# SuperScientificSoftwareLaboratory/DASP

Measured on AMD Instinct MI355X. Metric: SpMV GFLOP/s (f64), higher is better.
Workload: dtype f64; 1 GPU; HV15R synthetic stand-in (seeded; SuiteSparse dims/row statistics), A=1, x=1; rows=2017169, cols=2017169, nnz=275454726, partition=single GPU, generator_rev=26e32ff958e7, y_candidates=1

## Files before the change

### dasp_amd/csrc/spmv_device.hpp

```cpp
#pragma once
#include <hip/hip_runtime.h>

#include <cstdint>

#include "plan.hpp"
#include "device.hpp"

namespace dasp {

typedef double f64x4 __attribute__((ext_vector_type(4)));
typedef double f64x2 __attribute__((ext_vector_type(2)));
typedef float f32x4 __attribute__((ext_vector_type(4)));
typedef _Float16 f16x4 __attribute__((ext_vector_type(4)));
typedef int i32x4 __attribute__((ext_vector_type(4)));
typedef int i32x2 __attribute__((ext_vector_type(2)));
typedef unsigned short u16x4 __attribute__((ext_vector_type(4)));
typedef unsigned short u16x8 __attribute__((ext_vector_type(8)));
typedef const __attribute__((address_space(1))) unsigned char *gbyte_p;
typedef _Float16 f16x8 __attribute__((ext_vector_type(8)));


template <bool NT, class U>
__device__ __forceinline__ U ldg(const U *p)
{
    if constexpr (NT) return __builtin_nontemporal_load(p);
    else return *p;
}

template <int CTRL>
__device__ __forceinline__ double dpp_mov_f64(double v)
{
    int lo = __double2loint(v), hi = __double2hiint(v);
    lo = __builtin_amdgcn_update_dpp(lo, lo, CTRL, 0xf, 0xf, false);
    hi = __builtin_amdgcn_update_dpp(hi, hi, CTRL, 0xf, 0xf, false);
    return __hiloint2double(hi, lo);
}
template <int CTRL>
__device__ __forceinline__ float dpp_mov_f32(float v)
{
    return __int_as_float(__builtin_amdgcn_update_dpp(__float_as_int(v), __float_as_int(v), CTRL, 0xf, 0xf, false));
}
__device__ __forceinline__ double readlane_f64(double v, int l)
{
    int lo = __builtin_amdgcn_readlane(__double2loint(v), l);
    int hi = __builtin_amdgcn_readlane(__double2hiint(v), l);
    return __hiloint2double(hi, lo);
}
__device__ __forceinline__ double wave_sum(double v)
{
    v += dpp_mov_f64<0x128>(v);
    v += dpp_mov_f64<0x124>(v);
    v += dpp_mov_f64<0x122>(v);
    v += dpp_mov_f64<0x121>(v);
    return (readlane_f64(v, 0) + readlane_f64(v, 16)) + (readlane_f64(v, 32) + readlane_f64(v, 48));
}
__device__ __forceinline__ float wave_sum(float v)
{
    v += dpp_mov_f32<0x128>(v);
    v += dpp_mov_f32<0x124>(v);
    v += dpp_mov_f32<0x122>(v);
    v += dpp_mov_f32<0x121>(v);
    float a = __int_as_float(__builtin_amdgcn_readlane(__float_as_int(v), 0));
    float b = __int_as_float(__builtin_amdgcn_readlane(__float_as_int(v), 16));
    float c = __int_as_float(__builtin_amdgcn_readlane(__float_as_int(v), 32));
    float d = __int_as_float(__builtin_amdgcn_readlane(__float_as_int(v), 48));
    return (a + b) + (c + d);
}

template <bool K, class U>
__device__ __forceinline__ U tab(const U *p, int i)
{
    if constexpr (K) return reinterpret_cast<const __attribute__((address_space(4))) U *>(reinterpret_cast<uintptr_t>(p))[i];
    else return p[i];
}

#ifdef DASP_STAMPS
struct CallArgs { const DevArgs *plan; const void *x; void *y; int acc, ywt, stamp_launch; };
#else
struct CallArgs { const DevArgs *plan; const void *x; void *y; int acc, ywt; };
#endif
template <class U> __device__ __forceinline__ U *ldp(U *const *field)
{
    typedef __attribute__((address_space(1))) U *gptr;
    return (U *)*reinterpret_cast<const __attribute__((address_space(4))) gptr *>(reinterpret_cast<uintptr_t>(field));
}
__device__ __forceinline__ DevArgs load_args(const CallArgs &c)
{
    static_assert(sizeof(DevArgs) % 4 == 0, "DevArgs is a whole number of words");
    int w[sizeof(DevArgs) / 4];
#pragma unroll
    for (int i = 0; i < (int)(sizeof(DevArgs) / 4); ++i) w[i] = tab<true>(reinterpret_cast<const int *>(c.plan), i);
    DevArgs a;
    __builtin_memcpy(&a, w, sizeof a);
#define DASP_G(f) a.f = ldp(&c.plan->f)
    DASP_G(long_val); DASP_G(long_cid); DASP_G(long_cid16); DASP_G(long_base); DASP_G(piece_c16); DASP_G(piece_ptr); DASP_G(piece_dst); DASP_G(partial); DASP_G(multi_ptr); DASP_G(multi_dst);
    DASP_G(med_ptr); DASP_G(med_val); DASP_G(med_cid); DASP_G(med_cid16); DASP_G(med_base); DASP_G(med_cid8); DASP_G(med_c8ptr); DASP_G(med_shplane); DASP_G(med_shtab);
    DASP_G(irr_ptr); DASP_G(med_nt); DASP_G(irr_val); DASP_G(irr_cid); DASP_G(med_dst); DASP_G(win_cmin); DASP_G(win_len);
    DASP_G(short_val); DASP_G(short_cid); DASP_G(groups); DASP_G(order);
    DASP_G(rt_val); DASP_G(rt_cid); DASP_G(rt_ptr); DASP_G(rt_start); DASP_G(rt_mask);
#undef DASP_G
    a.x = c.x; a.y = c.y; a.acc = c.acc; a.ywt = c.ywt;
    return a;
}

template <int I, int N> struct LastLE {
    static __device__ __forceinline__ void run(const int (&arr)[N], int w, int &idx, int &val)
    {
        if constexpr (I < N) { const bool in = w >= arr[I]; idx = in ? I : idx; val = in ? arr[I] : val; LastLE<I + 1, N>::run(arr, w, idx, val); }
    }
};
template <int I, int N> struct PickPair {
    static __device__ __forceinline__ void run(const int (&arr)[N], int k, int &lo, int &hi)
    {
        if constexpr (I + 1 < N) { lo = k == I ? arr[I] : lo; hi = k == I ? arr[I + 1] : hi; PickPair<I + 1, N>::run(arr, k, lo, hi); }
    }
};

__device__ __forceinline__ int slot_of(const SlotMap &m, int t)
{
    const int p = t < m.split ? 0 : 1;
    const int u = p ? t - m.split : t;
    const int g = m.grp[p];
    return g ? m.base[p] + (u / g) * 2 * g + m.off[p] + u % g : m.base[p] + u;
}

template <class T> struct Tr;
template <> struct Tr<double> {
    using acc_t = f64x4; using part_t = double;
    static constexpr int CHUNK = 64, SHORT_ROWS = 128, BATCH = kMedBatch64, SHOT = kMedShot64, LONG_SHOT = kMedShot64;
};
template <> struct Tr<_Float16> {
    using acc_t = f32x4; using part_t = float;
    static constexpr int CHUNK = 256, SHORT_ROWS = 256, BATCH = kMedBatch16, SHOT = kMedShot16, LONG_SHOT = 2;
};
static_assert(Tr<double>::BATCH == kMedBatch64 && Tr<double>::SHOT == kMedShot64 && Tr<_Float16>::BATCH == kMedBatch16 &&
              Tr<_Float16>::SHOT == kMedShot16 && kMedBatch64 % 2 == 0 && kMedBatch16 % 2 == 0, "the packers' pairing rule (plan.hpp) follows the kernel's batches");

template <class T> struct Frag;
template <> struct Frag<double> { double a; int c; double b; };
template <> struct Frag<_Float16> { f16x4 a; i32x4 c; f16x4 b; };

template <bool NT>
__device__ __forceinline__ void frag_load_at(Frag<double> &f, const double *val, const int *cid, size_t at)
{
    f.a = ldg<NT>(val + at);
    f.c = ldg<NT>(cid + at);
}
template <bool NT>
__device__ __forceinline__ void frag_load_at(Frag<_Float16> &f, const _Float16 *val, const int *cid, size_t at)
{
    f.a = ldg<NT>(reinterpret_cast<const f16x4 *>(val + at));
    f.c = ldg<NT>(reinterpret_cast<const i32x4 *>(cid + at));
}
template <bool NT, class T>
__device__ __forceinline__ void frag_load(Frag<T> &f, const T *val, const int *cid, size_t e, int lane)
{
    frag_load_at<NT>(f, val, cid, e + (size_t)(Tr<T>::CHUNK / kWave) * lane);
}
template <class T>
struct XGlobal {
    const T *x;
    __device__ __forceinline__ T at(int c) const { return x[c < 0 ? 0 : c]; }
};
template <class T> using lds_cptr = const __attribute__((address_space(3))) T *;
template <class T> using glb_cptr = const __attribute__((address_space(1))) T *;
template <class T>
struct XLds {
    lds_cptr<T> xw; int cmin;
    __device__ __forceinline__ T at(int c) const { return xw[c < 0 ? 0 : c - cmin]; }
};
template <class T>
struct XHyb {
    lds_cptr<T> xw; glb_cptr<T> xg; int cmin; unsigned len;
    __device__ __forceinline__ T at(int c) const
    {
        const unsigned o = (unsigned)(c - cmin);
        T v;
        if (c < 0) v = (T)0;
        else if (o < len) v = xw[o];
        else v = xg[c];
        return v;
    }
};
template <class XV>
__device__ __forceinline__ void frag_gather(Frag<double> &f, const XV &xv)
{
    const double v = xv.at(f.c);
    f.b = f.c < 0 ? 0.0 : v;
}
template <class XV>
__device__ __forceinline__ void frag_gather(Frag<_Float16> &f, const XV &xv)
{
#pragma unroll
    for (int j = 0; j < 4; ++j) {
        const _Float16 v = xv.at(f.c[j]);
        f.b[j] = f.c[j] < 0 ? (_Float16)0 : v;
    }
}
__device__ __forceinline__ void frag_mfma(f64x4 &acc, const Frag<double> &f)
{
    acc = __builtin_amdgcn_mfma_f64_16x16x4f64(f.a, f.b, acc, 0, 0, 0);
}
__device__ __forceinline__ void frag_mfma(f32x4 &acc, const Frag<_Float16> &f)
{
    acc = __builtin_amdgcn_mfma_f32_16x16x16f16(f.a, f.b, acc, 0, 0, 0);
}


template <class T, bool NT>
struct ChunkSrc {
    static constexpr bool kPairs = false, kQuadIds = false;
    const T *val; const int *cid; size_t e0; int lane;
    template <bool PAIRED_OK = true> __device__ __forceinline__ void load(Frag<T> &f, int i) const { frag_load<NT>(f, val, cid, e0 + (size_t)i * Tr<T>::CHUNK, lane); }
    template <bool QUAD = false, class XV> __device__ __forceinline__ void gather(Frag<T> &f, int, const XV &x) const { frag_gather(f, x); }
};

template <class T, bool NT, bool N16 = false>
struct PieceSrc {
    static constexpr bool kPairs = false, kQuadIds = false;
    static constexpr int VPL = Tr<T>::CHUNK / kWave;
    const T *val; const int *cid; size_t e0; int lane, nfull, tail;
    const unsigned short *cid16 = nullptr; const int *base = nullptr;
    template <bool PAIRED_OK = true> __device__ __forceinline__ void load(Frag<T> &f, int i) const
    {
        if constexpr (N16) {
            const size_t at = i < nfull || VPL * lane < tail ? e0 + (size_t)i * Tr<T>::CHUNK + (size_t)(VPL * lane) : e0;
            if constexpr (VPL == 1) { f.a = ldg<NT>(val + at); f.c = (int)ldg<NT>(cid16 + at); }
            else {
                f.a = ldg<NT>(reinterpret_cast<const f16x4 *>(val + at));
                const i32x2 o = ldg<NT>(reinterpret_cast<const i32x2 *>(cid16 + at));
                f.c[0] = o[0]; f.c[1] = o[1];
            }
        } else {
            if (i < nfull) frag_load<NT>(f, val, cid, e0 + (size_t)i * Tr<T>::CHUNK, lane);
            else frag_load_at<NT>(f, val, cid, VPL * lane < tail ? e0 + (size_t)i * Tr<T>::CHUNK + (size_t)(VPL * lane) : e0);
        }
    }
    template <bool QUAD = false, class XV> __device__ __forceinline__ void gather(Frag<T> &f, int i, const XV &x) const
    {
        if constexpr (N16) {
            const int b = tab<true>(base, i);
            if constexpr (VPL == 1) { const unsigned o = (unsigned)f.c; f.c = o == kLongPad16 ? -1 : b + (int)o; }
            else {
                const unsigned lo = (unsigned)f.c[0], hi = (unsigned)f.c[1];
                const unsigned o[4] = {lo & 0xFFFFu, lo >> 16, hi & 0xFFFFu, hi >> 16};
#pragma unroll
                for (int q = 0; q < 4; ++q) f.c[q] = o[q] == kLongPad16 ? -1 : b + (int)o[q];
            }
        }
        if (i >= nfull) {
            const bool ok = VPL * lane < tail;
            if constexpr (VPL == 1) { f.c = ok ? f.c : -1; f.a = ok ? f.a : 0.0; }
            else {
#pragma unroll
                for (int j = 0; j < 4; ++j) { f.c[j] = ok ? f.c[j] : -1; f.a[j] = ok ? f.a[j] : (_Float16)0; }
            }
        }
        frag_gather(f, x);
    }
};

template <class T, bool NT, bool C16, bool PAIRS, bool C8, bool KT = false, bool REL = false, bool SH = false>
struct BlockSrc {
    static constexpr bool kPairs = PAIRS;
    static constexpr int VPL = Tr<T>::CHUNK / kWave;
    ChunkSrc<T, NT> reg; int nc;
    int npair;
    const unsigned short *cid16; const int *base; int c0;
    int relb;
    const unsigned char *c8; const unsigned short *w16; int n8;
    gbyte_p shn, shw; unsigned sh4l, shlane4;
    const T *ival; const int *icid; int t0, t1, kq;
    template <bool PAIRED_OK> __device__ __forceinline__ size_t at_of(int i) const
    {
        constexpr int CH = Tr<T>::CHUNK;
        if constexpr (!PAIRED_OK || !PAIRS) return reg.e0 + (size_t)i * CH + (size_t)VPL * reg.lane;
        const bool paired = i < npair;
        const size_t s = reg.e0 + (paired ? (size_t)(i & ~1) * CH + (size_t)(VPL * (i & 1)) : (size_t)i * CH);
        return s + (size_t)(paired ? 2 * VPL : VPL) * reg.lane;
    }
    __device__ __forceinline__ bool pairs_ok(int i0, int n) const { return i0 + n <= npair; }
    __device__ __forceinline__ void load2(Frag<T> &f0, Frag<T> &f1, int i) const
    {
        constexpr int CH = Tr<T>::CHUNK;
        const size_t at = reg.e0 + (size_t)i * CH + (size_t)(2 * VPL) * reg.lane;
        if constexpr (sizeof(T) == 8) {
            const f64x2 v = ldg<NT>(reinterpret_cast<const f64x2 *>(reg.val + at));
            f0.a = v[0]; f1.a = v[1];
            if constexpr (C16) {
                if constexpr (kQuadIds) {
                    if (i < n8) {
                        const unsigned r = ldg<NT>(reinterpret_cast<const unsigned short *>(c8 + (size_t)i * CH) + reg.lane);
                        const unsigned b0 = r & 0xFFu, b1 = r >> 8;
                        f0.c = (int)(b0 == 0xFFu ? 0xFFFFu : b0); f1.c = (int)(b1 == 0xFFu ? 0xFFFFu : b1);
                        return;
                    }
                }
                const unsigned r = ldg<NT>(reinterpret_cast<const unsigned *>((kQuadIds ? w16 : cid16) + at));
                f0.c = (int)(r & 0xFFFFu); f1.c = (int)(r >> 16);
            } else {
                const i32x2 c = ldg<NT>(reinterpret_cast<const i32x2 *>(reg.cid + at));
                f0.c = c[0]; f1.c = c[1];
            }
        } else {
            const f16x8 v = ldg<NT>(reinterpret_cast<const f16x8 *>(reg.val + at));
            f0.a = __builtin_shufflevector(v, v, 0, 1, 2, 3); f1.a = __builtin_shufflevector(v, v, 4, 5, 6, 7);
            if constexpr (C16) {
                const i32x4 o = ldg<NT>(reinterpret_cast<const i32x4 *>(cid16 + at));
                f0.c[0] = o[0]; f0.c[1] = o[1]; f1.c[0] = o[2]; f1.c[1] = o[3];
            } else {
                f0.c = ldg<NT>(reinterpret_cast<const i32x4 *>(reg.cid + at));
                f1.c = ldg<NT>(reinterpret_cast<const i32x4 *>(reg.cid + at + 4));
            }
        }
    }
    static constexpr bool kQuadIds = C8 && PAIRS && C16 && sizeof(T) == 8 && Tr<T>::BATCH == 4;
    __device__ __forceinline__ void load4(Frag<T> *f, int i) const
    {
        constexpr int CH = Tr<T>::CHUNK;
        const size_t at = reg.e0 + (size_t)i * CH + (size_t)2 * reg.lane;
        const f64x2 v0 = ldg<NT>(reinterpret_cast<const f64x2 *>(reg.val + at));
        const f64x2 v1 = ldg<NT>(reinterpret_cast<const f64x2 *>(reg.val + at + 2 * CH));
        f[0].a = v0[0]; f[1].a = v0[1]; f[2].a = v1[0]; f[3].a = v1[1];
        const bool narrow = i + 4 <= n8;
        gbyte_p pa, pb; unsigned lo4;
        if constexpr (SH) {
            pa = narrow ? shn + (size_t)((unsigned)i * sh4l) : shw + (size_t)((unsigned)i * (2u * sh4l));
            pb = narrow ? pa : pa + 4u * sh4l;
            lo4 = shlane4;
        } else {
            pa = narrow ? (gbyte_p)(c8 + (size_t)i * CH) : (gbyte_p)(w16 + reg.e0 + (size_t)i * CH);
            pb = narrow ? pa : pa + 4 * CH;
            lo4 = 4u * (unsigned)reg.lane;
        }
        const unsigned ra = ldg<NT>((const __attribute__((address_space(1))) unsigned *)(pa + lo4));
        const unsigned rb = ldg<NT>((const __attribute__((address_space(1))) unsigned *)(pb + lo4));
        f[0].c = (int)ra; f[1].c = (int)ra; f[2].c = (int)rb; f[3].c = (int)rb;
    }
    template <bool PAIRED_OK = true> __device__ __forceinline__ void load(Frag<T> &f, int i) const
    {
        if (i < nc) {
            const size_t at = at_of<PAIRED_OK>(i);
            if constexpr (!C16) frag_load_at<NT>(f, reg.val, reg.cid, at);
            else {
                if constexpr (sizeof(T) == 8) {
                    f.a = ldg<NT>(reg.val + at);
                    f.c = (int)ldg<NT>((kQuadIds ? w16 : cid16) + at);
                } else {
                    f.a = ldg<NT>(reinterpret_cast<const f16x4 *>(reg.val + at));
                    const i32x2 o = ldg<NT>(reinterpret_cast<const i32x2 *>(cid16 + at));
                    f.c[0] = o[0]; f.c[1] = o[1];
                }
            }
            return;
        }
        const int j = i - nc;
        if constexpr (sizeof(T) == 8) {
            const int e = t0 + 4 * j + kq;
            const int ee = e < t1 ? e : 0;
            f.a = ldg<NT>(ival + ee);
            f.c = ldg<NT>(icid + ee);
        } else {
#pragma unroll
            for (int q = 0; q < 4; ++q) {
                const int e = t0 + 16 * j + 4 * kq + q;
                const int ee = e < t1 ? e : 0;
                f.a[q] = ival[ee];
                f.c[q] = icid[ee];
            }
        }
    }
    template <bool QUAD = false, class XV> __device__ __forceinline__ void gather(Frag<T> &f, int i, const XV &x) const
    {
        if (i >= nc) {
            const int j = i - nc;
            if constexpr (sizeof(T) == 8) {
                const bool ok = t0 + 4 * j + kq < t1;
                f.a = ok ? f.a : 0.0;
                f.c = ok ? f.c : -1;
            } else {
#pragma unroll
                for (int q = 0; q < 4; ++q) {
                    const bool ok = t0 + 16 * j + 4 * kq + q < t1;
                    f.a[q] = ok ? f.a[q] : (_Float16)0;
                    f.c[q] = ok ? f.c[q] : -1;
                }
            }
        } else if constexpr (C16) {
            const int b = REL ? relb : tab<KT>(base, c0 + i);
            if constexpr (sizeof(T) == 8) {
                unsigned o = (unsigned)f.c, pad = 0xFFFFu;
                if constexpr (QUAD && kQuadIds) {
                    const bool narrow = i < n8, paired = i < npair;
                    pad = narrow ? 0xFFu : 0xFFFFu;
                    o = (o >> (narrow ? 8u * (i & 3) : (paired ? 16u * (i & 1) : 0u))) & pad;
                }
                f.c = o == pad ? -1 : b + (int)o;
            }
            else {
                const unsigned lo = (unsigned)f.c[0], hi = (unsigned)f.c[1];
                const unsigned o[4] = {lo & 0xFFFFu, lo >> 16, hi & 0xFFFFu, hi >> 16};
#pragma unroll
                for (int q = 0; q < 4; ++q) f.c[q] = o[q] == 0xFFFFu ? -1 : b + (int)o[q];
            }
        }
        frag_gather(f, x);
    }
};

template <int N, class SRC, class T>
__device__ __forceinline__ void load_steps(const SRC &src, Frag<T> *f, int i0)
{
    if constexpr (SRC::kPairs && N == Tr<T>::BATCH) {
        if (src.pairs_ok(i0, N)) {
            if constexpr (SRC::kQuadIds) src.load4(f, i0);
            else {
#pragma unroll
                for (int u = 0; u < N; u += 2) src.load2(f[u], f[u + 1], i0 + u);
            }
            return;
        }
    }
#pragma unroll
    for (int u = 0; u < N; ++u) src.load(f[u], i0 + u);
}

template <class T, int N, class SRC, class ACC, class XV>
__device__ __forceinline__ void shot(ACC &acc, const SRC &src, int i0, const XV &x)
{
    Frag<T> f[N];
    if constexpr (SRC::kPairs && sizeof(T) == 2) {
#pragma unroll
        for (int u = 0; u + 1 < N; u += 2) {
            if (src.pairs_ok(i0 + u, 2)) src.load2(f[u], f[u + 1], i0 + u);
            else { src.load(f[u], i0 + u); src.load(f[u + 1], i0 + u + 1); }
        }
        if constexpr (N % 2 == 1) src.load(f[N - 1], i0 + N - 1);
    } else if constexpr (SRC::kPairs && N >= 2) {
        if (src.pairs_ok(i0, N & ~1)) {
#pragma unroll
            for (int u = 0; u + 1 < N; u += 2) src.load2(f[u], f[u + 1], i0 + u);
            if constexpr (N % 2 == 1) src.template load<false>(f[N - 1], i0 + N - 1);
        } else {
#pragma unroll
            for (int u = 0; u < N; ++u) src.template load<false>(f[u], i0 + u);
        }
    } else {
#pragma unroll
        for (int u = 0; u < N; ++u) src.template load<false>(f[u], i0 + u);
    }
#pragma unroll
    for (int u = 0; u < N; ++u) src.gather(f[u], i0 + u, x);
#pragma unroll
    for (int u = 0; u < N; ++u) frag_mfma(acc, f[u]);
}
template <class T, int N, class SRC, class ACC, class XV>
struct ShotDispatch {
    static __device__ __forceinline__ void run(ACC &acc, const SRC &src, int i0, int n, const XV &x)
    {
        if (n == N) shot<T, N>(acc, src, i0, x);
        else ShotDispatch<T, N - 1, SRC, ACC, XV>::run(acc, src, i0, n, x);
    }
};
template <class T, class SRC, class ACC, class XV>
struct ShotDispatch<T, 0, SRC, ACC, XV> {
    static __device__ __forceinline__ void run(ACC &, const SRC &, int, int, const XV &) {}
};

template <class T, int U, int R, class SRC, class ACC, class XV>
struct FinishDispatch {
    static __device__ __forceinline__ void run(ACC &acc, const SRC &src, Frag<T> (&cur)[U], int ibase, int i, int rem, const XV &x)
    {
        if (rem == R) {
            Frag<T> r[R > 0 ? R : 1];
#pragma unroll
            for (int u = 0; u < U; ++u) src.template gather<true>(cur[u], ibase + u, x);
            load_steps<R>(src, r, i);
#pragma unroll
            for (int u = 0; u < U; ++u) frag_mfma(acc, cur[u]);
#pragma unroll
            for (int u = 0; u < R; ++u) src.template gather<true>(r[u], i + u, x);
#pragma unroll
            for (int u = 0; u < R; ++u) frag_mfma(acc, r[u]);
        } else if constexpr (R > 0) FinishDispatch<T, U, R - 1, SRC, ACC, XV>::run(acc, src, cur, ibase, i, rem, x);
    }
};

template <class T, int U, int S, class SRC, class ACC, class XV>
__device__ __forceinline__ void run_stream(ACC &acc, const SRC &src, int N, const XV &x)
{
    if (N <= S) { ShotDispatch<T, S, SRC, ACC, XV>::run(acc, src, 0, N, x); return; }
    const int nfull = N / U, rem = N % U;
    Frag<T> cur[U];
    load_steps<U>(src, cur, 0);
    int i = U;
    for (int it = 1; it < nfull; ++it, i += U) {
        Frag<T> nxt[U];
#pragma unroll
        for (int u = 0; u < U; ++u) src.template gather<true>(cur[u], i - U + u, x);
        load_steps<U>(src, nxt, i);
#pragma unroll
        for (int u = 0; u < U; ++u) frag_mfma(acc, cur[u]);
#pragma unroll
        for (int u = 0; u < U; ++u) cur[u] = nxt[u];
    }
    FinishDispatch<T, U, U - 1, SRC, ACC, XV>::run(acc, src, cur, i - U, i, rem, x);
}

template <class T, int YS = 0, class P>
__device__ __forceinline__ void put_y(const DevArgs &a, int yi, P v)
{
    T *y = static_cast<T *>(a.y) + yi;
    if constexpr (YS == 1) *(volatile T *)y = (T)v;
    else if constexpr (YS == 2) {
        const T old = *(volatile T *)y;
        *(volatile T *)y = (T)((P)old + v);
    }
    else if (a.acc) *y = (T)((P)*y + v);
    else if (a.ywt) *(volatile T *)y = (T)v;
    else *y = (T)v;
}

__device__ __forceinline__ bool diag_of(const f64x4 &acc, int lane, double &d)
{
    const int r = (lane & 15) >> 2;
    d = r == 0 ? acc[0] : r == 1 ? acc[1] : r == 2 ? acc[2] : acc[3];
    return (lane & 3) == (lane >> 4);
}
__device__ __forceinline__ bool diag_of(const f32x4 &acc, int lane, float &d)
{
    const int r = lane & 3;
    d = r == 0 ? acc[0] : r == 1 ? acc[1] : r == 2 ? acc[2] : acc[3];
    return ((lane & 15) >> 2) == (lane >> 4);
}

template <class T, bool NT, bool C16, int YM, bool C8 = false, int YS = 0, bool REL = false, int WU = 0, int WS = 0, bool SH = false, class XV>
__device__ __forceinline__ void medium_block(const DevArgs &a, int b, int lane, const XV &x)
{
    using acc_t = typename Tr<T>::acc_t;
    constexpr int CH = Tr<T>::CHUNK;
    const T *val = static_cast<const T *>(a.med_val);
    constexpr bool KT = true;
    const int c0 = tab<KT>(a.med_ptr, b), c1 = tab<KT>(a.med_ptr, b + 1);
    acc_t acc = {0, 0, 0, 0};
    const int row = lane & 15, kq = lane >> 4;
    const int r = b * kMedRows + row;
    int t0 = 0, t1 = 0;
    if (r < a.row_block) { t0 = a.irr_ptr[r]; t1 = a.irr_ptr[r + 1]; }
    constexpr int TK = sizeof(T) == 8 ? 4 : 16;
    const int nt = YS == 0 ? tab<true>(a.med_nt, b) : (__builtin_amdgcn_readfirstlane(t1 - t0) + TK - 1) / TK;
    BlockSrc<T, NT, C16, YM != 2, C8, KT, REL, SH> src;
    if constexpr (REL) src.relb = x.cmin; else src.relb = 0;
    src.reg.val = val; src.reg.cid = a.med_cid; src.reg.e0 = (size_t)c0 * CH; src.reg.lane = lane;
    src.nc = c1 - c0; src.npair = med_npair(c1 - c0, nt, (int)sizeof(T), YM == 2 ? 0 : a.pair_mode); src.cid16 = a.med_cid16; src.base = a.med_base; src.c0 = c0;
    src.c8 = a.med_cid8; src.w16 = a.med_cid16; src.n8 = 0;
    if constexpr (C8 && C16 && sizeof(T) == 8 && YM != 2) {
        const int q0 = tab<true>(a.med_c8ptr, b), q1 = tab<true>(a.med_c8ptr, b + 1);
        src.n8 = q1 - q0; src.c8 = a.med_cid8 + (size_t)q0 * CH; src.w16 = a.med_cid16 - (size_t)q1 * CH;
    }
    if constexpr (SH) {
        static_assert(C8 && C16 && sizeof(T) == 8 && YM == 0, "the shared id plane belongs to the one-byte-id f64 build");
        typedef unsigned u32x4 __attribute__((ext_vector_type(4)));
        const u32x4 e = tab<true>(reinterpret_cast<const u32x4 *>(a.med_shtab), b);
        const unsigned L = e[3], rw = row < 8 ? e[0] : e[1];
        src.sh4l = 4u * L; src.shlane4 = 4u * ((unsigned)kq * L + ((rw >> (4u * (unsigned)(row & 7))) & 15u));
        src.shn = (gbyte_p)a.med_shplane + (size_t)e[2] * 16;
        src.shw = src.shn - (size_t)((unsigned)src.n8 * src.sh4l);
    }
    src.ival = static_cast<const T *>(a.irr_val); src.icid = a.irr_cid; src.t0 = t0; src.t1 = t1; src.kq = kq;
    run_stream<T, (WU > 0 && sizeof(T) == 8) ? WU : Tr<T>::BATCH, (YM == 2 && sizeof(T) == 2) ? 2 : ((WS > 0 && sizeof(T) == 8) ? WS : Tr<T>::SHOT)>(acc, src, src.nc + nt, x);

    typename Tr<T>::part_t d;
    if (diag_of(acc, lane, d) && r < a.row_block) {
        const int slot = a.row_long + r;
        const int yi = YM == 2 ? a.med_dst[r] : (a.order ? a.order[slot] : slot);
        put_y<T, YS>(a, yi, d);
    }
}

template <class T, bool NT, int YS = 0, bool TAIL_IN = false, bool L16 = false>
__device__ __forceinline__ void long_piece(const DevArgs &a, int p, int lane)
{
    using acc_t = typename Tr<T>::acc_t;
    using part_t = typename Tr<T>::part_t;
    constexpr int CH = Tr<T>::CHUNK;
    constexpr int VPL = CH / kWave;
    const XGlobal<T> x{static_cast<const T *>(a.x)};
    const T *val = static_cast<const T *>(a.long_val);
    const int p0 = tab<true>(a.piece_ptr, p), p1 = tab<true>(a.piece_ptr, p + 1);
    acc_t acc = {0, 0, 0, 0};
    const int nfull = (p1 - p0) / CH, tail = (p1 - p0) - nfull * CH;
    bool narrow = false;
    if constexpr (L16) narrow = tab<true>(a.piece_c16, 2 * p + 1) != 0;
    if (L16 && narrow) {
        const PieceSrc<T, NT, true> src{val, a.long_cid, (size_t)p0, lane, nfull, tail, a.long_cid16, a.long_base + tab<true>(a.piece_c16, 2 * p)};
        run_stream<T, Tr<T>::BATCH, Tr<T>::LONG_SHOT>(acc, src, nfull + (tail > 0 ? 1 : 0), x);
    } else if (TAIL_IN && tail > 0) {
        const PieceSrc<T, NT> src{val, a.long_cid, (size_t)p0, lane, nfull, tail};
        run_stream<T, Tr<T>::BATCH, Tr<T>::LONG_SHOT>(acc, src, nfull + 1, x);
    } else {
        const int full = p0 + nfull * CH;
        ChunkSrc<T, NT> src{val, a.long_cid, (size_t)p0, lane};
        run_stream<T, Tr<T>::BATCH, Tr<T>::LONG_SHOT>(acc, src, nfull, x);
        if (full < p1) {
            const int i = full + VPL * lane;
            const bool ok = i < p1;
            Frag<T> f;
            frag_load_at<NT>(f, val, a.long_cid, (size_t)(ok ? i : p0));
            frag_gather(f, x);
            if constexpr (VPL == 1) { f.a = ok ? f.a : 0.0; f.b = ok ? f.b : 0.0; }
            else {
#pragma unroll
                for (int j = 0; j < 4; ++j) { f.a[j] = ok ? f.a[j] : (_Float16)0; f.b[j] = ok ? f.b[j] : (_Float16)0; }
            }
            frag_mfma(acc, f);
        }
    }
    part_t d;
    const bool on_diag = diag_of(acc, lane, d);
    const part_t total = wave_sum(on_diag ? d : (part_t)0);
    if (lane == 0) {
        const int dst = tab<true>(a.piece_dst, p);
        if (dst >= 0) put_y<T, YS>(a, dst, total);
        else static_cast<part_t *>(a.partial)[~dst] = total;
    }
}

template <class T, int L, bool NT, int YS = 0>
__device__ __forceinline__ void short_rows(const DevArgs &a, const ShortDev &g, int local_tile, int lane)
{
    constexpr int SR = Tr<T>::SHORT_ROWS;
    constexpr int V = SR / kWave;
    const T *x = static_cast<const T *>(a.x);
    const T *val = static_cast<const T *>(a.short_val);
    using part_t = typename Tr<T>::part_t;
    part_t s[V];
#pragma unroll
    for (int v = 0; v < V; ++v) s[v] = 0;
    const size_t base = (size_t)g.elem_off + (size_t)local_tile * L * SR + (size_t)V * lane;
#pragma unroll
    for (int k = 0; k < L; ++k) {
        if constexpr (V == 2) {
            const f64x2 av = ldg<NT>(reinterpret_cast<const f64x2 *>(val + base + (size_t)k * SR));
            const i32x2 c = ldg<NT>(reinterpret_cast<const i32x2 *>(a.short_cid + base + (size_t)k * SR));
            const double x0 = x[c[0] < 0 ? 0 : c[0]], x1 = x[c[1] < 0 ? 0 : c[1]];
            s[0] += av[0] * (c[0] < 0 ? 0.0 : x0);
            s[1] += av[1] * (c[1] < 0 ? 0.0 : x1);
        } else {
            const f16x4 av = ldg<NT>(reinterpret_cast<const f16x4 *>(val + base + (size_t)k * SR));
            const i32x4 c = ldg<NT>(reinterpret_cast<const i32x4 *>(a.short_cid + base + (size_t)k * SR));
#pragma unroll
            for (int v = 0; v < 4; ++v) {
                const _Float16 xv = x[c[v] < 0 ? 0 : c[v]];
                s[v] += (float)av[v] * (c[v] < 0 ? 0.0f : (float)xv);
            }
        }
    }
    const int t0 = local_tile * SR + V * lane;
#pragma unroll
    for (int v = 0; v < V; ++v) {
        const int t = t0 + v;
        if (t < g.count) {
            const int slot = slot_of(g.map, t);
            const int yi = a.order ? a.order[slot] : slot;
            put_y<T, YS>(a, yi, s[v]);
        }
    }
}

template <class T, int L, bool NT, int YS = 0>
__device__ __forceinline__ void short_rows_seg(const DevArgs &a, const ShortDev &g, int local_tile, int lane)
{
    constexpr int PER16 = 16 / L, RPW = 4 * PER16;
    using part_t = typename Tr<T>::part_t;
    const T *x = static_cast<const T *>(a.x);
    const int sub = lane & 15, rloc = sub / L, k = sub - rloc * L;
    const int t = local_tile * RPW + (lane >> 4) * PER16 + rloc;
    const size_t e = (size_t)g.elem_off + (size_t)local_tile * kWave + (size_t)lane;
    const T av = ldg<NT>(static_cast<const T *>(a.short_val) + e);
    const int c = ldg<NT>(a.short_cid + e);
    const T xv = x[c < 0 ? 0 : c];
    part_t p = c < 0 ? (part_t)0 : (part_t)av * (part_t)xv;
    if constexpr (L >= 2) {
        part_t q;
        if constexpr (sizeof(part_t) == 8) q = dpp_mov_f64<0x101>(p); else q = dpp_mov_f32<0x101>(p);
        if (k + 1 < L) p += q;
    }
    if constexpr (L >= 3) {
        part_t q;
        if constexpr (sizeof(part_t) == 8) q = dpp_mov_f64<0x102>(p); else q = dpp_mov_f32<0x102>(p);
        if (k == 0) p += q;
    }
    if (k == 0 && rloc < PER16 && t < g.count) {
        const int slot = slot_of(g.map, t);
        const int yi = a.order ? a.order[slot] : slot;
        put_y<T, YS>(a, yi, p);
    }
}

template <class T, int L, bool NT, int TPW>
__device__ __forceinline__ void short_rows_seg_multi(const DevArgs &a, const ShortDev &g, int local0, int nv, int lane)
{
    constexpr int PER16 = 16 / L, RPW = 4 * PER16;
    using part_t = typename Tr<T>::part_t;
    const T *x = static_cast<const T *>(a.x);
    const int sub = lane & 15, rloc = sub / L, k = sub - rloc * L;
    T av[TPW]; int c[TPW]; T xv[TPW];
#pragma unroll
    for (int u = 0; u < TPW; ++u) {
        const size_t e = (size_t)g.elem_off + (size_t)(local0 + (u < nv ? u : 0)) * kWave + (size_t)lane;
        av[u] = ldg<NT>(static_cast<const T *>(a.short_val) + e);
        c[u] = ldg<NT>(a.short_cid + e);
    }
#pragma unroll
    for (int u = 0; u < TPW; ++u) xv[u] = x[c[u] < 0 ? 0 : c[u]];
#pragma unroll
    for (int u = 0; u < TPW; ++u) {
        part_t p = c[u] < 0 ? (part_t)0 : (part_t)av[u] * (part_t)xv[u];
        if constexpr (L >= 2) {
            part_t q;
            if constexpr (sizeof(part_t) == 8) q = dpp_mov_f64<0x101>(p); else q = dpp_mov_f32<0x101>(p);
            if (k + 1 < L) p += q;
        }
        if constexpr (L >= 3) {
            part_t q;
            if constexpr (sizeof(part_t) == 8) q = dpp_mov_f64<0x102>(p); else q = dpp_mov_f32<0x102>(p);
            if (k == 0) p += q;
        }
        const int t = (local0 + u) * RPW + (lane >> 4) * PER16 + rloc;
        if (u < nv && k == 0 && rloc < PER16 && t < g.count) {
            const int slot = slot_of(g.map, t);
            const int yi = a.order ? a.order[slot] : slot;
            put_y<T>(a, yi, p);
        }
    }
}

template <class T, bool NT, int YS = 0>
__device__ __forceinline__ void slab_rows(const DevArgs &a, const ShortDev &g, int local_tile, int lane)
{
    constexpr int SR = Tr<T>::SHORT_ROWS;
    constexpr int V = SR / kWave;
    const T *x = static_cast<const T *>(a.x);
    const T *val = static_cast<const T *>(a.short_val);
    using part_t = typename Tr<T>::part_t;
    const int L = g.len;
    part_t s[V];
#pragma unroll
    for (int v = 0; v < V; ++v) s[v] = 0;
    const size_t base = (size_t)g.elem_off + (size_t)local_tile * L * SR + (size_t)V * lane;
#pragma unroll 4
    for (int k = 0; k < L; ++k) {
        if constexpr (V == 2) {
            const f64x2 av = ldg<NT>(reinterpret_cast<const f64x2 *>(val + base + (size_t)k * SR));
            const i32x2 c = ldg<NT>(reinterpret_cast<const i32x2 *>(a.short_cid + base + (size_t)k * SR));
            const double x0 = x[c[0] < 0 ? 0 : c[0]], x1 = x[c[1] < 0 ? 0 : c[1]];
            s[0] += av[0] * (c[0] < 0 ? 0.0 : x0);
            s[1] += av[1] * (c[1] < 0 ? 0.0 : x1);
        } else {
            const f16x4 av = ldg<NT>(reinterpret_cast<const f16x4 *>(val + base + (size_t)k * SR));
            const i32x4 c = ldg<NT>(reinterpret_cast<const i32x4 *>(a.short_cid + base + (size_t)k * SR));
#pragma unroll
            for (int v = 0; v < 4; ++v) {
                const _Float16 xv = x[c[v] < 0 ? 0 : c[v]];
                s[v] += (float)av[v] * (c[v] < 0 ? 0.0f : (float)xv);
            }
        }
    }
    const int t0 = local_tile * SR + V * lane;
#pragma unroll
    for (int v = 0; v < V; ++v) {
        const int t = t0 + v;
        if (t < g.count) {
            const int slot = g.map.base[0] + t;
            const int yi = a.order ? a.order[slot] : slot;
            put_y<T, YS>(a, yi, s[v]);
        }
    }
}

template <class T, bool NT, int YS = 0, bool SEG = true>
__device__ __forceinline__ void short_tile(const DevArgs &a, int tile, int lane)
{
    int gi = 0, t0_unused = 0;
    LastLE<1, kNumShortGroups>::run(a.grp_tile0, tile, gi, t0_unused);
    ShortDev g;
    if constexpr (YS != 0) {
        static_assert(sizeof(ShortDev) % 4 == 0, "ShortDev is a whole number of words");
        int w[sizeof(ShortDev) / 4];
#pragma unroll
        for (int i = 0; i < (int)(sizeof(ShortDev) / 4); ++i) w[i] = tab<true>(reinterpret_cast<const int *>(a.groups + gi), i);
        __builtin_memcpy(&g, w, sizeof g);
    } else g = a.groups[gi];
    const int local = tile - g.tile0;
    if constexpr (SEG) {
        if (g.seg) {
            switch (g.len) {
                case 1: short_rows_seg<T, 1, NT, YS>(a, g, local, lane); break;
                case 2: short_rows_seg<T, 2, NT, YS>(a, g, local, lane); break;
                case 3: short_rows_seg<T, 3, NT, YS>(a, g, local, lane); break;
                default: short_rows_seg<T, 4, NT, YS>(a, g, local, lane); break;
            }
            return;
        }
    }
    switch (g.len) {
        case 0: if constexpr (YS != 2) { if (!a.skip0 && !a.acc) short_rows<T, 0, NT, YS>(a, g, local, lane); } break;
        case 1: short_rows<T, 1, NT, YS>(a, g, local, lane); break;
        case 2: short_rows<T, 2, NT, YS>(a, g, local, lane); break;
        case 3: short_rows<T, 3, NT, YS>(a, g, local, lane); break;
        case 4: short_rows<T, 4, NT, YS>(a, g, local, lane); break;
        default: slab_rows<T, NT, YS>(a, g, local, lane); break;
    }
}

template <class T, bool NT, int TPW>
__device__ __forceinline__ void short_waves(const DevArgs &a, int w, int lane)
{
    int gi = 0, w0 = 0;
    LastLE<1, kNumShortGroups>::run(a.grp_wave0, w, gi, w0);
    const ShortDev g = a.groups[gi];
    const int lw = w - w0;
    if (!g.seg) { short_tile<T, NT, 0, false>(a, g.tile0 + lw, lane); return; }
    const int local0 = lw * TPW, nv = min(TPW, g.tiles - local0);
    switch (g.len) {
        case 1: short_rows_seg_multi<T, 1, NT, TPW>(a, g, local0, nv, lane); break;
        case 2: short_rows_seg_multi<T, 2, NT, TPW>(a, g, local0, nv, lane); break;
        case 3: short_rows_seg_multi<T, 3, NT, TPW>(a, g, local0, nv, lane); break;
        default: short_rows_seg_multi<T, 4, NT, TPW>(a, g, local0, nv, lane); break;
    }
}

template <class T, bool NT>
__device__ __forceinline__ void row_tile(const DevArgs &a, int t, int lane, typename Tr<T>::part_t *prod)
{
    using part_t = typename Tr<T>::part_t;
    const T *x = static_cast<const T *>(a.x), *val = static_cast<const T *>(a.rt_val);
    const int e0 = a.rt_ptr[t], n = a.rt_ptr[t + 1] - e0;
    const int s = a.rt_start[(size_t)t * kRowTile + lane];
#pragma unroll 4
    for (int i = lane; i < n; i += kWave) prod[i] = (part_t)ldg<NT>(val + e0 + i) * (part_t)x[ldg<NT>(a.rt_cid + e0 + i)];
    int e = __shfl_down(s, 1);
    if (lane == kWave - 1) e = n;
    part_t sum = 0;
    for (int j = s; j < e; ++j) sum += prod[j];
    if ((a.rt_mask[t] >> lane) & 1) put_y<T>(a, t * kRowTile + lane, sum);
}

#ifdef DASP_STAMPS
struct StampBuf { unsigned long long *rec; unsigned cap; };
static __device__ StampBuf g_stamps;
struct Stamps {
    unsigned long long wall0, clk[4];
    int kind, launch;
    __device__ __forceinline__ void begin(int launch_no) { wall0 = __builtin_amdgcn_s_memrealtime(); clk[0] = __builtin_readcyclecounter(); clk[1] = clk[2] = clk[3] = clk[0]; kind = 0; launch = launch_no; }
    __device__ __forceinline__ void mark(int i) { asm volatile("s_waitcnt vmcnt(0) lgkmcnt(0)" ::: "memory"); clk[i] = __builtin_readcyclecounter(); }
    __device__ __forceinline__ void finish(int nwaves)
    {
        asm volatile("s_waitcnt vmcnt(0) lgkmcnt(0)" ::: "memory");
        const unsigned long long e = __builtin_readcyclecounter();
        const unsigned long long wall1 = __builtin_amdgcn_s_memrealtime();
        const size_t slot = ((size_t)launch * gridDim.x + blockIdx.x) * (size_t)nwaves + (threadIdx.x >> 6);
        if ((threadIdx.x & 63) == 0 && g_stamps.rec && launch >= 0 && slot < g_stamps.cap) {
            unsigned long long *r = g_stamps.rec + slot * 12;
            unsigned xcc, hw;
            asm volatile("s_getreg_b32 %0, hwreg(HW_REG_XCC_ID)" : "=s"(xcc));
            asm volatile("s_getreg_b32 %0, hwreg(HW_REG_HW_ID)" : "=s"(hw));
            r[0] = blockIdx.x | ((unsigned long long)(threadIdx.x >> 6) << 32) | ((unsigned long long)nwaves << 40) | ((unsigned long long)kind << 48) | (1ull << 63);
            r[1] = xcc | ((unsigned long long)hw << 32); r[2] = gridDim.x; r[3] = wall0; r[4] = wall1;
            r[5] = clk[0]; r[6] = clk[1]; r[7] = clk[2]; r[8] = clk[3]; r[9] = e; r[10] = (unsigned long long)launch; r[11] = 0;
        }
    }
};
#else
struct Stamps {
    int kind;
    __device__ __forceinline__ void begin(int) {}
    __device__ __forceinline__ void mark(int) {}
};
#endif

#ifndef DASP_MIN_WAVES
#define DASP_MIN_WAVES 1
#endif
constexpr int kMinWavesPlain = DASP_MIN_WAVES, kMinWavesWin = 8;
#ifndef DASP_WIN64_U
#define DASP_WIN64_U 3
#define DASP_WIN64_S 6
#endif
template <class T, bool NT, bool C16, bool WIN, bool C8, bool RT = false, bool W64 = false, bool L16 = false, bool SH = false>
__device__ __forceinline__ void spmv_body(const DevArgs &a, char *lds_raw, int wg_index, Stamps &st)
{
    const int lane = threadIdx.x & 63;
    const int wave = __builtin_amdgcn_readfirstlane(threadIdx.x >> 6);
    int wg = wg_index;
    if constexpr (sizeof(T) == 2 && !WIN && !RT) {
        if (a.wg_rot) { const int grid = a.wg_long + a.wg_med + a.wg_short; wg += a.wg_rot; wg = wg >= grid ? wg - grid : wg; }
    }
    const int wpw = WIN ? a.wpw : kWavesPerWG;
    if (wg < a.wg_long) {
        const int p = wg * wpw + wave;
        if (p < a.n_pieces) long_piece<T, NT, 0, !WIN, L16 && !WIN>(a, p, lane);
    } else if (wg < a.wg_long + a.wg_med) {
        st.kind = 1;
        if constexpr (!WIN) {
            const int m = wg - a.wg_long;
            const XGlobal<T> x{static_cast<const T *>(a.x)};
            if (a.xcd_on) {
                const int k = m & 7;
                int lo = a.xcd_blk[0], hi = a.xcd_blk[1];
                PickPair<1, 9>::run(a.xcd_blk, k, lo, hi);
                const int b = lo + (m >> 3) * kWavesPerWG + wave;
                if (b < hi) medium_block<T, NT, C16, 0, C8, 0, false, 0, 0, SH>(a, b, lane, x);
            } else if (sizeof(T) == 8 && !a.med_stride) {
                const int b = m * kWavesPerWG + wave;
                if (b < a.n_blocks) medium_block<T, NT, C16, 0, C8, 0, false, 0, 0, SH>(a, b, lane, x);
            } else {
#pragma unroll 1
            for (int b = m * kWavesPerWG + wave; b < a.n_blocks; b += a.wg_med * kWavesPerWG)
                medium_block<T, NT, C16, 0, C8, 0, false, 0, 0, SH>(a, b, lane, x);
            }
        } else {
            const int mw = wg - a.wg_long, per_xcd = a.wg_med >> 3;
            const int w = a.win_xcd ? (mw & 7) * per_xcd + (mw >> 3) : mw;
            if (w >= a.n_windows) return;
            const int len = a.win_len[w], cmin = a.win_cmin[w];
            const T *xg = static_cast<const T *>(a.x);
            __shared__ int next_unit_word;
            int *next_unit = &next_unit_word;
            typedef __attribute__((address_space(3))) T lds_T;
            lds_T *xw = (lds_T *)lds_raw;
            if (threadIdx.x == 0) *next_unit = wpw;
            st.kind = 3; st.mark(1);
            if (len > 0) {
                constexpr int A = 16 / (int)sizeof(T);
                const i32x4 *src = reinterpret_cast<const i32x4 *>(xg + cmin);
                typedef __attribute__((address_space(3))) i32x4 lds_i32x4;
                lds_i32x4 *dst = (lds_i32x4 *)xw;
                const int nvec = len / A, nth = wpw * kWave;
                for (int i0 = threadIdx.x; i0 < nvec; i0 += 4 * nth) {
                    const int i1 = i0 + nth, i2 = i0 + 2 * nth, i3 = i0 + 3 * nth;
                    const i32x4 v0 = src[i0];
                    const i32x4 v1 = src[i1 < nvec ? i1 : i0], v2 = src[i2 < nvec ? i2 : i0], v3 = src[i3 < nvec ? i3 : i0];
                    dst[i0] = v0;
                    if (i1 < nvec) dst[i1] = v1;
                    if (i2 < nvec) dst[i2] = v2;
                    if (i3 < nvec) dst[i3] = v3;
                }
                for (int i = nvec * A + threadIdx.x; i < len; i += nth) xw[i] = xg[cmin + i];
                st.mark(2);
            }
            __syncthreads();
            st.mark(3);
            const int n_units = a.blocks_per_win + a.win_tiles;
            constexpr int WU = W64 ? DASP_WIN64_U : 0, WS = W64 ? DASP_WIN64_S : 0;
            int q = wave;
#define DASP_NEXT_UNIT()                                                                                          \
            {                                                                                                     \
                int nq = 0;                                                                                       \
                if (lane == 0) nq = atomicAdd(next_unit, 1);                                                      \
                q = __builtin_amdgcn_readfirstlane(nq);                                                           \
            }
#define DASP_WINDOW_BLOCKS(BLOCK_CALL)                                                                            \
            while (q < a.blocks_per_win) {                                                                        \
                const int b = w * a.blocks_per_win + q;                                                           \
                if (b < a.n_blocks) { BLOCK_CALL; }                                                               \
                DASP_NEXT_UNIT()                                                                                  \
            }
            if (len > 0) {
                if (a.win_hybrid) {
                    const XHyb<T> x{xw, (glb_cptr<T>)xg, cmin, (unsigned)len};
                    DASP_WINDOW_BLOCKS((medium_block<T, NT, C16, 2, false, 0, false, WU, WS>(a, b, lane, x)))
                } else if (C16 && a.win_rel16) {
                    const XLds<T> x{xw, cmin};
#ifdef DASP_WIN_KEEPMOD
                    if ((w % DASP_WIN_KEEPMOD) != DASP_WIN_KEEPMOD - 1) { DASP_WINDOW_BLOCKS((medium_block<T, false, C16, 2, false, 0, C16, WU, WS>(a, b, lane, x))) }
                    else
#endif
                    DASP_WINDOW_BLOCKS((medium_block<T, NT, C16, 2, false, 0, C16, WU, WS>(a, b, lane, x)))
                } else {
                    const XLds<T> x{xw, cmin};
                    DASP_WINDOW_BLOCKS((medium_block<T, NT, C16, 2, false, 0, false, WU, WS>(a, b, lane, x)))
                }
            } else {
                const XGlobal<T> x{xg};
                DASP_WINDOW_BLOCKS((medium_block<T, NT, C16, 2, false, 0, false, WU, WS>(a, b, lane, x)))
            }
            while (q < n_units) {
                const int t = w + (q - a.blocks_per_win) * a.n_windows;
                if (t < a.n_short_tiles) short_tile<T, NT, 0, false>(a, t, lane);
                DASP_NEXT_UNIT()
            }
#undef DASP_WINDOW_BLOCKS
#undef DASP_NEXT_UNIT
        }
    } else if (!RT || wg < a.wg_long + a.wg_med + a.wg_short) {
        st.kind = 2;
        const int t = (wg - a.wg_long - a.wg_med) * wpw + wave;
        if constexpr (!WIN && sizeof(T) == 8) {
            if (a.short_tpw > 1) {
                if (t < a.n_short_waves) short_waves<T, NT, kShortTpw>(a, t, lane);
                return;
            }
        }
        if (t < a.n_short_tiles) short_tile<T, NT, 0, !WIN>(a, t, lane);
    } else if constexpr (RT) {
        const int t = (wg - a.wg_long - a.wg_med - a.wg_short) * kWavesPerWG + wave;
        if (t < a.n_rt_tiles) row_tile<T, NT>(a, t, lane, reinterpret_cast<typename Tr<T>::part_t *>(lds_raw) + (size_t)wave * kRowTile * a.rt_max);
    }
}

template <class T, bool NT, bool C16, bool C8, int YS>
__device__ __forceinline__ void plain_wg(const DevArgs &a, int wg, int wave, int lane, const int *blk_order)
{
    if (wg < a.wg_long) {
        const int p = wg * kWavesPerWG + wave;
        if (p < a.n_pieces) long_piece<T, NT, YS>(a, p, lane);
    } else if (wg < a.wg_long + a.wg_med) {
        const int q = (wg - a.wg_long) * kWavesPerWG + wave;
        const XGlobal<T> x{static_cast<const T *>(a.x)};
        if (q < a.n_blocks) medium_block<T, NT, C16, 0, C8, YS>(a, blk_order ? tab<true>(blk_order, q) : q, lane, x);
    } else {
        const int t = (wg - a.wg_long - a.wg_med) * kWavesPerWG + wave;
        if (t < a.n_short_tiles) short_tile<T, NT, YS, YS == 0>(a, t, lane);
    }
}

}
```

Measured before the change: 1283 GFLOP/s.

## Add deep software-pipelined stream for shared-id-plane medium blocks

```diff
diff --git a/dasp_amd/csrc/spmv_device.hpp b/dasp_amd/csrc/spmv_device.hpp
--- a/dasp_amd/csrc/spmv_device.hpp
+++ b/dasp_amd/csrc/spmv_device.hpp
@@ -209,7 +209,7 @@
 
 template <class T, bool NT>
 struct ChunkSrc {
-    static constexpr bool kPairs = false, kQuadIds = false;
+    static constexpr bool kPairs = false, kQuadIds = false, kDeep = false;
     const T *val; const int *cid; size_t e0; int lane;
     template <bool PAIRED_OK = true> __device__ __forceinline__ void load(Frag<T> &f, int i) const { frag_load<NT>(f, val, cid, e0 + (size_t)i * Tr<T>::CHUNK, lane); }
     template <bool QUAD = false, class XV> __device__ __forceinline__ void gather(Frag<T> &f, int, const XV &x) const { frag_gather(f, x); }
@@ -217,7 +217,7 @@
 
 template <class T, bool NT, bool N16 = false>
 struct PieceSrc {
-    static constexpr bool kPairs = false, kQuadIds = false;
+    static constexpr bool kPairs = false, kQuadIds = false, kDeep = false;
     static constexpr int VPL = Tr<T>::CHUNK / kWave;
     const T *val; const int *cid; size_t e0; int lane, nfull, tail;
     const unsigned short *cid16 = nullptr; const int *base = nullptr;
@@ -260,7 +260,7 @@
     }
 };
 
-template <class T, bool NT, bool C16, bool PAIRS, bool C8, bool KT = false, bool REL = false, bool SH = false>
+template <class T, bool NT, bool C16, bool PAIRS, bool C8, bool KT = false, bool REL = false, bool SH = false, bool DEEP = SH>
 struct BlockSrc {
     static constexpr bool kPairs = PAIRS;
     static constexpr int VPL = Tr<T>::CHUNK / kWave;
@@ -337,6 +337,34 @@
         const unsigned rb = ldg<NT>((const __attribute__((address_space(1))) unsigned *)(pb + lo4));
         f[0].c = (int)ra; f[1].c = (int)ra; f[2].c = (int)rb; f[3].c = (int)rb;
     }
+    static constexpr bool kDeep = SH && DEEP;
+    __device__ __forceinline__ void load4_val(Frag<T> *f, int i) const
+    {
+        constexpr int CH = Tr<T>::CHUNK;
+        const size_t at = reg.e0 + (size_t)i * CH + (size_t)2 * reg.lane;
+        const f64x2 v0 = ldg<NT>(reinterpret_cast<const f64x2 *>(reg.val + at));
+        const f64x2 v1 = ldg<NT>(reinterpret_cast<const f64x2 *>(reg.val + at + 2 * CH));
+        f[0].a = v0[0]; f[1].a = v0[1]; f[2].a = v1[0]; f[3].a = v1[1];
+    }
+    __device__ __forceinline__ void load4_id(Frag<T> *f, int i) const
+    {
+        static_assert(SH, "the deep stream reads the shared plane");
+        const bool narrow = i + 4 <= n8;
+        const gbyte_p pa = narrow ? shn + (size_t)((unsigned)i * sh4l) : shw + (size_t)((unsigned)i * (2u * sh4l));
+        const gbyte_p pb = narrow ? pa : pa + 4u * sh4l;
+        const unsigned ra = ldg<NT>((const __attribute__((address_space(1))) unsigned *)(pa + shlane4));
+        const unsigned rb = ldg<NT>((const __attribute__((address_space(1))) unsigned *)(pb + shlane4));
+        f[0].c = (int)ra; f[1].c = (int)ra; f[2].c = (int)rb; f[3].c = (int)rb;
+    }
+    template <class XV> __device__ __forceinline__ void gather_paired(Frag<T> &f, int i, const XV &x) const
+    {
+        const int b = REL ? relb : tab<KT>(base, c0 + i);
+        const bool narrow = i < n8;
+        const unsigned pad = narrow ? 0xFFu : 0xFFFFu;
+        const unsigned o = ((unsigned)f.c >> (narrow ? 8u * (i & 3) : 16u * (i & 1))) & pad;
+        f.c = o == pad ? -1 : b + (int)o;
+        frag_gather(f, x);
+    }
     template <bool PAIRED_OK = true> __device__ __forceinline__ void load(Frag<T> &f, int i) const
     {
         if (i < nc) {
@@ -486,10 +514,71 @@
     }
 };
 
+__device__ __forceinline__ double keep_copy(double v)
+{
+    const long long b = __builtin_bit_cast(long long, v);
+    const unsigned lo = (unsigned)__builtin_amdgcn_update_dpp(0, (int)(unsigned)b, 0xE4, 0xF, 0xF, false);
+    const unsigned hi = (unsigned)__builtin_amdgcn_update_dpp(0, (int)(unsigned)(b >> 32), 0xE4, 0xF, 0xF, false);
+    return __builtin_bit_cast(double, (long long)(((unsigned long long)hi << 32) | lo));
+}
+
+template <class T, int U, bool FAR, class ACC, class SRC, class XV>
+__device__ __forceinline__ void deep_step(ACC &acc, const SRC &src, Frag<T> (&p)[U], Frag<T> (&q)[U], Frag<T> (&r)[U], int k, const XV &x)
+{
+    Frag<T> g[U];
+#pragma unroll
+    for (int u = 0; u < U; ++u) { g[u].a = p[u].a; g[u].c = p[u].c; src.gather_paired(g[u], k * U + u, x); }
+    src.load4_id(q, (k + 1) * U);
+    __builtin_amdgcn_sched_barrier(0xF);
+    if constexpr (FAR) src.load4_val(r, (k + 2) * U);
+#pragma unroll
+    for (int u = 0; u < U; ++u) frag_mfma(acc, g[u]);
+#pragma unroll
+    for (int u = 0; u < U; ++u) { p[u].a = keep_copy(q[u].a); p[u].c = q[u].c; }
+    __builtin_amdgcn_sched_barrier(0);
+}
+
+template <class T, int U, class SRC, class ACC, class XV>
+__device__ __forceinline__ void run_stream_deep(ACC &acc, const SRC &src, int N, const XV &x)
+{
+    const int nfull = N / U, rem = N % U;
+    Frag<T> cur[U];
+    int i = U, it = 1;
+    {
+        const int nb = src.npair / U;
+        if (nb >= 3) {
+            Frag<T> b1[U], b2[U];
+            src.load4_id(cur, 0); src.load4_val(cur, 0); src.load4_val(b1, U);
+            int k = 0;
+            for (; k + 2 <= nb - 2; k += 2) {
+                deep_step<T, U, true>(acc, src, cur, b1, b2, k, x);
+                deep_step<T, U, true>(acc, src, cur, b2, b1, k + 1, x);
+            }
+            if (k < nb - 2) {
+                deep_step<T, U, true>(acc, src, cur, b1, b2, k, x);
+                deep_step<T, U, false>(acc, src, cur, b2, b1, k + 1, x);
+            } else deep_step<T, U, false>(acc, src, cur, b1, b2, k, x);
+            it = nb; i = nb * U;
+        } else load_steps<U>(src, cur, 0);
+    }
+    for (; it < nfull; ++it, i += U) {
+        Frag<T> nxt[U];
+#pragma unroll
+        for (int u = 0; u < U; ++u) src.template gather<true>(cur[u], i - U + u, x);
+        load_steps<U>(src, nxt, i);
+#pragma unroll
+        for (int u = 0; u < U; ++u) frag_mfma(acc, cur[u]);
+#pragma unroll
+        for (int u = 0; u < U; ++u) cur[u] = nxt[u];
+    }
+    FinishDispatch<T, U, U - 1, SRC, ACC, XV>::run(acc, src, cur, i - U, i, rem, x);
+}
+
 template <class T, int U, int S, class SRC, class ACC, class XV>
 __device__ __forceinline__ void run_stream(ACC &acc, const SRC &src, int N, const XV &x)
 {
     if (N <= S) { ShotDispatch<T, S, SRC, ACC, XV>::run(acc, src, 0, N, x); return; }
+    if constexpr (SRC::kDeep) { run_stream_deep<T, U>(acc, src, N, x); return; }
     const int nfull = N / U, rem = N % U;
     Frag<T> cur[U];
     load_steps<U>(src, cur, 0);
@@ -534,7 +623,7 @@
     return ((lane & 15) >> 2) == (lane >> 4);
 }
 
-template <class T, bool NT, bool C16, int YM, bool C8 = false, int YS = 0, bool REL = false, int WU = 0, int WS = 0, bool SH = false, class XV>
+template <class T, bool NT, bool C16, int YM, bool C8 = false, int YS = 0, bool REL = false, int WU = 0, int WS = 0, bool SH = false, bool DEEP = SH, class XV>
 __device__ __forceinline__ void medium_block(const DevArgs &a, int b, int lane, const XV &x)
 {
     using acc_t = typename Tr<T>::acc_t;
@@ -549,7 +638,7 @@
     if (r < a.row_block) { t0 = a.irr_ptr[r]; t1 = a.irr_ptr[r + 1]; }
     constexpr int TK = sizeof(T) == 8 ? 4 : 16;
     const int nt = YS == 0 ? tab<true>(a.med_nt, b) : (__builtin_amdgcn_readfirstlane(t1 - t0) + TK - 1) / TK;
-    BlockSrc<T, NT, C16, YM != 2, C8, KT, REL, SH> src;
+    BlockSrc<T, NT, C16, YM != 2, C8, KT, REL, SH, DEEP> src;
     if constexpr (REL) src.relb = x.cmin; else src.relb = 0;
     src.reg.val = val; src.reg.cid = a.med_cid; src.reg.e0 = (size_t)c0 * CH; src.reg.lane = lane;
     src.nc = c1 - c0; src.npair = med_npair(c1 - c0, nt, (int)sizeof(T), YM == 2 ? 0 : a.pair_mode); src.cid16 = a.med_cid16; src.base = a.med_base; src.c0 = c0;
@@ -918,7 +1007,7 @@
             } else {
 #pragma unroll 1
             for (int b = m * kWavesPerWG + wave; b < a.n_blocks; b += a.wg_med * kWavesPerWG)
-                medium_block<T, NT, C16, 0, C8, 0, false, 0, 0, SH>(a, b, lane, x);
+                medium_block<T, NT, C16, 0, C8, 0, false, 0, 0, SH, false>(a, b, lane, x);
             }
         } else {
             const int mw = wg - a.wg_long, per_xcd = a.wg_med >> 3;
```

After: 1296 GFLOP/s (median of 6 runs). 1.01x the previous value.
